# usc-isi/PipeEdge

Measured on NVIDIA H100. Metric: images/sec per pipeline, higher is better.
Workload: dtype f16

## Files before the change

### pipeedge_b200/csrc/gemm_wgmma.cu

```cuda
#include <math.h>
#include <stdio.h>
#include <stdlib.h>

#include "../../include/pipeedge_b200.h"
#include "common.cuh"
#include "ln_dev.cuh"
#include "wgmma.cuh"

namespace pe {

void count_launches(int n);
int require_sm90();

constexpr int kBlockM = 128;
constexpr int kBlockK = 64;
constexpr int kMmaK = 16;
constexpr int kNumConsumerWarps = 8;
constexpr int kConsumerThreads = kNumConsumerWarps * 32;
constexpr int kProducerWarp = kNumConsumerWarps;
constexpr int kWeightWarp = kNumConsumerWarps + 1;
constexpr int kGemmThreads = (kNumConsumerWarps + 2) * 32;
constexpr int kMaxStages = 8;
constexpr int kTraceSlots = 32;
constexpr int kPipeSmemBudget = 144 * 1024;
constexpr int kABytes = kBlockM * kBlockK * 2;

struct GemmParams {
  const float* bias;
  const float* resid;
  void* out;
  int m, n, k;
  int block_n;
  int stages;
  int num_m_blocks, num_n_blocks, num_k_blocks;
  long long* trace;
  int cm, cn;
  int num_super_m, num_super_n;
  int rows_per_item;
  int out_item_rows;
  int out_row_offset;
  int resid_per_item;
  int stg_offset;
  int static_w;
  int tma_out;
  const float* ln_gamma;
  const float* ln_beta;
  float ln_eps;
  int ln_off;
  int f32_is_ln;
  __half* out16;
};

constexpr int kLnAreaBytes = 8192;

__device__ __forceinline__ float gelu_erf(float x) { return 0.5f * x * (1.0f + erff(x * 0.70710678118654752f)); }
__device__ __forceinline__ float gelu_erf_fast(float x) {
  const float a = fminf(fabsf(x), 6.0f);
  float pl = fmaf(-1.889626233e-06f, a, 6.268140101e-05f);
  pl = fmaf(pl, a, -9.388679333e-04f);
  pl = fmaf(pl, a, 8.539461332e-03f);
  pl = fmaf(pl, a, -5.402068712e-02f);
  pl = fmaf(pl, a, -4.584097768e-01f);
  pl = fmaf(pl, a, -1.151269147e+00f);
  pl = fmaf(pl, a, -9.999943403e-01f);
  float e;
  asm("ex2.approx.ftz.f32 %0, %1;" : "=f"(e) : "f"(pl));
  return fmaxf(x, 0.0f) - fabsf(x * e);
}

constexpr int kStgLd = 36;
constexpr int kLnLdPad = 4;
constexpr int kStgBytesPerWarp = 16 * (128 + kLnLdPad) * 4;
constexpr int kStgBytes = kNumConsumerWarps * kStgBytesPerWarp;

__device__ __forceinline__ void map_rows(const GemmParams& p, int row, int& out_row, int& resid_row) {
  out_row = row;
  resid_row = row;
  if (p.rows_per_item > 0) {
    const int item = row / p.rows_per_item;
    const int in_item = row - item * p.rows_per_item + p.out_row_offset;
    out_row = item * p.out_item_rows + in_item;
    resid_row = p.resid_per_item ? in_item : out_row;
  }
}

template <int EPI>
__device__ __forceinline__ float epi_act(float x) {
  if (EPI == PE_EPI_GELU_F16) return gelu_erf_fast(x);
  if (EPI == PE_EPI_TANH_F32) return tanhf(x);
  return x;
}

template <int EPI>
__device__ __forceinline__ void epilogue_chunk16(const GemmParams& p, const float* stg, int row0, int col0, int lane) {
  constexpr bool kHalfOut = (EPI == PE_EPI_F16 || EPI == PE_EPI_GELU_F16);
  const bool vec_ok = (p.n & 7) == 0;
  if (kHalfOut) {
// ... 47 lines not shown
        if (row < p.m && fast) {
          int out_row, resid_row;
          map_rows(p, row, out_row, resid_row);
          res[it] = *reinterpret_cast<const float4*>(p.resid + static_cast<size_t>(resid_row) * p.n + col);
        }
      }
    }
    float4 bias4 = make_float4(0.f, 0.f, 0.f, 0.f);
    if (p.bias != nullptr && fast) bias4 = __ldg(reinterpret_cast<const float4*>(p.bias + col));
#pragma unroll
    for (int it = 0; it < 4; ++it) {
      const int rr = it * 4 + (lane >> 3);
      const int row = row0 + rr;
      if (row >= p.m || !col_ok) continue;
      int out_row, resid_row;
      map_rows(p, row, out_row, resid_row);
      const float4 a = *reinterpret_cast<const float4*>(stg + rr * kStgLd + cc);
      float* o = reinterpret_cast<float*>(p.out) + static_cast<size_t>(out_row) * p.n + col;
      if (fast) {
        float4 r4;
        r4.x = epi_act<EPI>(a.x + bias4.x) + res[it].x;
        r4.y = epi_act<EPI>(a.y + bias4.y) + res[it].y;
        r4.z = epi_act<EPI>(a.z + bias4.z) + res[it].z;
        r4.w = epi_act<EPI>(a.w + bias4.w) + res[it].w;
        *reinterpret_cast<float4*>(o) = r4;
      } else {
        const float v[4] = {a.x, a.y, a.z, a.w};
        for (int i = 0; i < 4 && col + i < p.n; ++i) {
          float x = v[i];
          if (p.bias != nullptr) x += __ldg(p.bias + col + i);
          x = epi_act<EPI>(x);
          if (EPI == PE_EPI_RESID_F32) x += p.resid[static_cast<size_t>(resid_row) * p.n + col + i];
          o[i] = x;
        }
      }
    }
  }
}

template <int J, int NACC>
__device__ __forceinline__ void stage_fragment(const float (&acc)[NACC], int j0, float* dst, int ld, int lane) {
  const int r = lane >> 2, c = (lane & 3) * 2;
#pragma unroll
  for (int j = 0; j < J; ++j) {
    *reinterpret_cast<float2*>(dst + r * ld + 8 * j + c) = make_float2(acc[4 * (j0 + j)], acc[4 * (j0 + j) + 1]);
    *reinterpret_cast<float2*>(dst + (r + 8) * ld + 8 * j + c) = make_float2(acc[4 * (j0 + j) + 2], acc[4 * (j0 + j) + 3]);
  }
}

constexpr int kWgStgBytes = 4 * kStgBytesPerWarp;
constexpr int kWgBoxBytes = 32 * 1024;
constexpr int kOutBoxCols = 32;

template <int EPI, int BN>
__device__ __forceinline__ void epilogue_tma(const GemmParams& p, const CUtensorMap* tm_c, const CUtensorMap* tm_r,
                                             const float (&acc)[BN / 2], uint8_t* stg, uint32_t stg_addr,
                                             uint32_t res_bar, uint32_t& res_phase, int row_wg, int col_tile, int wg,
                                             int lane, bool issuer) {
  constexpr bool kHalfOut = (EPI == PE_EPI_F16 || EPI == PE_EPI_GELU_F16);
  constexpr int kRowBytes = kOutBoxCols * (kHalfOut ? 2 : 4);
  constexpr int kBoxBytes = 64 * kRowBytes;
  constexpr int kBoxes = BN / kOutBoxCols;
  constexpr int kPass = kBoxes < kWgBoxBytes / kBoxBytes ? kBoxes : kWgBoxBytes / kBoxBytes;
  static_assert(kWgBoxBytes + 256 * 4 <= kWgStgBytes, "boxes + bias exceed a warpgroup's staging");
  float* bias_s = reinterpret_cast<float*>(stg + kWgBoxBytes);
  const int t = threadIdx.x & 127;
  const int r0 = (t >> 5) * 16 + (lane >> 2);
  const int cq = (lane & 3) * 2;
#pragma unroll
  for (int b0 = 0; b0 < kBoxes; b0 += kPass) {
    if (issuer) {
      tma_store_wait_read();
      if (EPI == PE_EPI_RESID_F32) {
        const int nb = (kBoxes - b0 < kPass ? kBoxes - b0 : kPass);
        int boxes = 0;
        if (row_wg < p.m)
          for (int b = 0; b < nb && col_tile + (b0 + b) * kOutBoxCols < p.n; ++b) boxes = b + 1;
        mbar_arrive_expect_tx_addr(res_bar, static_cast<uint32_t>(boxes * kBoxBytes));
        for (int b = 0; b < boxes; ++b)
          tma_load_2d_addr(stg_addr + static_cast<uint32_t>(b * kBoxBytes), tm_r, res_bar,
                           col_tile + (b0 + b) * kOutBoxCols, row_wg);
      }
    }
    if (b0 == 0) {
      for (int c = t; c < BN; c += 128) {
        const int col = col_tile + c;
        bias_s[c] = p.bias != nullptr && col < p.n ? __ldg(p.bias + col) : 0.f;
      }
    }
    named_barrier_id(3 + wg, 128);
    if (EPI == PE_EPI_RESID_F32) {
      mbar_wait_addr(res_bar, res_phase);
      res_phase ^= 1u;
    }
#pragma unroll
    for (int i = 0; i < kPass * 4; ++i) {
      const int j = b0 * 4 + i, jj = i & 3;
      if (j >= BN / 8) break;
      const float2 bv = *reinterpret_cast<const float2*>(bias_s + 8 * j + cq);
      uint8_t* box = stg + (i >> 2) * kBoxBytes;
#pragma unroll
      for (int h = 0; h < 2; ++h) {
        const int r = r0 + 8 * h;
        const float x0 = acc[4 * j + 2 * h] + bv.x, x1 = acc[4 * j + 2 * h + 1] + bv.y;
        if (kHalfOut) {
          *reinterpret_cast<__half2*>(box + r * kRowBytes + ((jj ^ ((r >> 1) & 3)) << 4) + cq * 2) =
              __floats2half2_rn(epi_act<EPI>(x0), epi_act<EPI>(x1));
        } else {
          float2* o = reinterpret_cast<float2*>(box + r * kRowBytes + (((2 * jj + (lane & 3) / 2) ^ (r & 7)) << 4) +
                                                (lane & 1) * 8);
          const float2 rv = EPI == PE_EPI_RESID_F32 ? *o : make_float2(0.f, 0.f);
          *o = make_float2(epi_act<EPI>(x0) + rv.x, epi_act<EPI>(x1) + rv.y);
        }
      }
    }
    fence_proxy_async_smem();
    named_barrier_id(3 + wg, 128);
    if (issuer) {
      if (row_wg < p.m) {
#pragma unroll
        for (int b = 0; b < kPass; ++b) {
          const int col = col_tile + (b0 + b) * kOutBoxCols;
          if (b0 + b < kBoxes && col < p.n) tma_store_2d(tm_c, stg_addr + static_cast<uint32_t>(b * kBoxBytes), col, row_wg);
        }
      }
      tma_store_commit();
    }
  }
}

template <int EPI, int BN>
__global__ void __launch_bounds__(kGemmThreads, 1)
gemm_wgmma_kernel(const __grid_constant__ CUtensorMap tm_a, const __grid_constant__ CUtensorMap tm_b,
                  const __grid_constant__ CUtensorMap tm_c, const __grid_constant__ CUtensorMap tm_r,
                  const GemmParams p) {
  extern __shared__ uint8_t smem_raw[];
  __shared__ __align__(8) uint64_t full_bar[kMaxStages];
  __shared__ __align__(8) uint64_t empty_bar[kMaxStages];
  __shared__ __align__(8) uint64_t ln_bar[2];
  __shared__ __align__(8) uint64_t res_bar[2];

  const int warp = threadIdx.x >> 5;
  const int lane = threadIdx.x & 31;
  long long* trace = p.trace != nullptr ? p.trace + static_cast<size_t>(blockIdx.x) * kTraceSlots : nullptr;
  if (trace != nullptr && threadIdx.x == 0) trace[0] = clock64();
  pdl_launch_dependents();
  const uint32_t smem_base = (smem_u32(smem_raw) + 1023u) & ~1023u;
  uint8_t* smem_gen = smem_raw + (smem_base - smem_u32(smem_raw));
  constexpr uint32_t stage_bytes = kABytes + static_cast<uint32_t>(BN) * (kBlockK * 2);

  const int csize = p.cm * p.cn;
  const uint32_t crank = csize > 1 ? cluster_ctarank() : 0u;
  const int m_rank = static_cast<int>(crank) % p.cm;
  const int n_rank = static_cast<int>(crank) / p.cm;
  uint16_t row_mask = 0, col_mask = 0;
  for (int c = 0; c < p.cn; ++c) row_mask |= static_cast<uint16_t>(1u << (m_rank + p.cm * c));
  for (int m = 0; m < p.cm; ++m) col_mask |= static_cast<uint16_t>(1u << (m + p.cm * n_rank));
  const uint16_t peers_mask = row_mask | col_mask;

  if (warp == kProducerWarp && lane == 0) {
    tma_prefetch_desc(&tm_a);
    tma_prefetch_desc(&tm_b);
    if (p.tma_out) tma_prefetch_desc(&tm_c);
    if (p.tma_out && EPI == PE_EPI_RESID_F32) tma_prefetch_desc(&tm_r);
    for (int s = 0; s < p.stages; ++s) {
      mbar_init(&full_bar[s], 1);
      mbar_init(&empty_bar[s], static_cast<uint32_t>(2 * (p.cm + p.cn - 1)));
    }
    for (int s = 0; s < 2; ++s) mbar_init(&ln_bar[s], static_cast<uint32_t>(p.cn));
    for (int s = 0; s < 2; ++s) mbar_init(&res_bar[s], 1);
    fence_barrier_init();
  }
  __syncthreads();
  if (csize > 1) cluster_sync_all();
  if (warp != kWeightWarp || p.static_w == 0) pdl_wait();
  if (trace != nullptr && threadIdx.x == 0) trace[1] = clock64();
  const int num_supers = p.num_super_m * p.num_super_n;
  const int cluster_id = static_cast<int>(blockIdx.x) / csize;
  const int num_clusters = static_cast<int>(gridDim.x) / csize;
  const int a_slice_rows = kBlockM / p.cn;
  const int b_slice_rows = p.block_n / p.cm;

  const uint32_t full_addr0 = keep_in_register(smem_u32(&full_bar[0]));
  const uint32_t empty_addr0 = keep_in_register(smem_u32(&empty_bar[0]));
  const int num_k_blocks = p.num_k_blocks, num_stages = p.stages;
  if (warp == kProducerWarp) {
    const int cm = p.cm, cn = p.cn, nsm = p.num_super_m;
    const uint32_t a_off = static_cast<uint32_t>(n_rank * a_slice_rows) * (kBlockK * 2);
    int stage = 0;
    uint32_t phase = 0;
    for (int sup = cluster_id; sup < num_supers; sup += num_clusters) {
      const int a_row = ((sup % nsm) * cm + m_rank) * kBlockM + n_rank * a_slice_rows;
      for (int kb = 0; kb < num_k_blocks; ++kb) {
        mbar_wait_addr(empty_addr0 + static_cast<uint32_t>(stage) * 8u, phase ^ 1u);
        if (elect_one()) {
          const uint32_t f = full_addr0 + static_cast<uint32_t>(stage) * 8u;
          const uint32_t sa = smem_base + static_cast<uint32_t>(stage) * stage_bytes + a_off;
          mbar_arrive_expect_tx_addr(f, stage_bytes);
          if (cn > 1) tma_load_2d_multicast_addr(sa, &tm_a, f, kb * kBlockK, a_row, row_mask);
          else tma_load_2d_addr(sa, &tm_a, f, kb * kBlockK, a_row);
        }
        __syncwarp();
        if (++stage == num_stages) { stage = 0; phase ^= 1u; }
      }
    }
  } else if (warp == kWeightWarp) {
    const int cm = p.cm, cn = p.cn, nsm = p.num_super_m, bn = p.block_n;
    const uint32_t b_off = kABytes + static_cast<uint32_t>(m_rank * b_slice_rows) * (kBlockK * 2);
    if (p.static_w != 0 && cluster_id < num_supers && elect_one()) {
      const int b_row = ((cluster_id / nsm) * cn + n_rank) * bn + m_rank * b_slice_rows;
      const int sharers = nsm * cm;
      const int me = (cluster_id % nsm) * cm + m_rank;
      for (int kb = num_stages + me; kb < num_k_blocks; kb += sharers) tma_prefetch_l2_2d(&tm_b, kb * kBlockK, b_row);
    }
    __syncwarp();
    int stage = 0;
    uint32_t phase = 0;
    for (int sup = cluster_id; sup < num_supers; sup += num_clusters) {
      const int b_row = ((sup / nsm) * cn + n_rank) * bn + m_rank * b_slice_rows;
      for (int kb = 0; kb < num_k_blocks; ++kb) {
        mbar_wait_addr(empty_addr0 + static_cast<uint32_t>(stage) * 8u, phase ^ 1u);
        if (elect_one()) {
          const uint32_t f = full_addr0 + static_cast<uint32_t>(stage) * 8u;
          const uint32_t sb = smem_base + static_cast<uint32_t>(stage) * stage_bytes + b_off;
          if (cm > 1) tma_load_2d_multicast_addr(sb, &tm_b, f, kb * kBlockK, b_row, col_mask);
          else tma_load_2d_addr(sb, &tm_b, f, kb * kBlockK, b_row);
        }
        __syncwarp();
        if (++stage == num_stages) { stage = 0; phase ^= 1u; }
      }
    }
  } else {
    const int wg = warp >> 2;
    const uint32_t a_wg_off = static_cast<uint32_t>(wg * 64) * (kBlockK * 2);
    const bool releaser = (warp & 3) == 0 && lane < csize && ((peers_mask >> lane) & 1u) != 0;
    const uint32_t empty_remote0 =
        csize > 1 ? mapa_shared(empty_addr0, static_cast<uint32_t>(lane < csize ? lane : 0)) : empty_addr0;
    float* stg = reinterpret_cast<float*>(smem_gen + p.stg_offset + warp * kStgBytesPerWarp);
    const bool store_issuer = (threadIdx.x & 127) == 0;
    const uint32_t res_bar_addr = smem_u32(&res_bar[wg]);
    uint32_t res_phase = 0u;
    int stage = 0;
    uint32_t phase = 0;
    int par = 0;
    uint32_t ln_phases = 0u;
    for (int sup = cluster_id; sup < num_supers; sup += num_clusters) {
      const int m_blk = (sup % p.num_super_m) * p.cm + m_rank;
      const int n_blk = (sup / p.num_super_m) * p.cn + n_rank;
      const int tslot = trace == nullptr || threadIdx.x != 0 ? -1 : (sup == cluster_id ? 0 : (sup == cluster_id + num_clusters ? 5 : -1));
      float acc[BN / 2];
#pragma unroll
      for (int i = 0; i < BN / 2; ++i) acc[i] = 0.f;
      int prev_stage = -1;
      for (int kb = 0; kb < num_k_blocks; ++kb) {
        mbar_wait_addr(full_addr0 + static_cast<uint32_t>(stage) * 8u, phase);
        if (tslot >= 0 && kb == 0) trace[2 + tslot] = clock64();
        const uint32_t sa = smem_base + static_cast<uint32_t>(stage) * stage_bytes;
        const uint64_t da = wgmma_desc_kmajor_sw128(sa + a_wg_off);
        const uint64_t db = wgmma_desc_kmajor_sw128(sa + kABytes);
        wgmma_fence();
#pragma unroll
        for (int k = 0; k < kBlockK / kMmaK; ++k)
          Wgmma<BN>::mma(acc, da + 2 * k, db + 2 * k, (kb | k) != 0 ? 1u : 0u);
        wgmma_commit();
        wgmma_wait<1>();
        if (prev_stage >= 0 && releaser) {
          const uint32_t e = empty_remote0 + static_cast<uint32_t>(prev_stage) * 8u;
          if (csize > 1) mbar_arrive_remote(e);
          else mbar_arrive_addr(e);
        }
        prev_stage = stage;
        if (++stage == num_stages) { stage = 0; phase ^= 1u; }
      }
      wgmma_wait<0>();
      if (releaser) {
        const uint32_t e = empty_remote0 + static_cast<uint32_t>(prev_stage) * 8u;
        if (csize > 1) mbar_arrive_remote(e);
        else mbar_arrive_addr(e);
      }
      if (tslot >= 0) trace[3 + tslot] = clock64();
      if (p.stg_offset == 0) named_barrier<1>(kConsumerThreads);
      const int row0 = m_blk * kBlockM + warp * 16;
      if (EPI == PE_EPI_RESID_LN) {
        constexpr int kLd = BN + kLnLdPad;
        constexpr int kChunks = BN / 32;
        float2* ln_part = reinterpret_cast<float2*>(smem_gen + p.ln_off);
        float2* ln_cta = ln_part + 4 * kBlockM;
        float2* ln_row = ln_cta + 2 * kBlockM;
        const int r_cta = warp * 16;
        const int gcol0 = n_blk * BN;
        stage_fragment<BN / 8>(acc, 0, stg, kLd, lane);
        __syncwarp();
        for (int idx = lane; idx < 16 * kChunks; idx += 32) {
          const int r = idx & 15, c = idx >> 4;
          const int row = row0 + r, gcol = gcol0 + c * 32;
          float* vr = stg + r * kLd + c * 32;
          float v[32];
          if (row < p.m) {
            const float4* r4 = reinterpret_cast<const float4*>(p.resid + static_cast<size_t>(row) * p.n + gcol);
            const float4* b4 = reinterpret_cast<const float4*>(p.bias + gcol);
#pragma unroll
            for (int i = 0; i < 8; ++i) {
// ... 12 lines not shown
          for (int i = 0; i < 8; ++i)
            *reinterpret_cast<float4*>(vr + 4 * i) = make_float4(v[4 * i], v[4 * i + 1], v[4 * i + 2], v[4 * i + 3]);
          float mean_c, m2_c;
          ln_chunk32(v, mean_c, m2_c);
          ln_part[(r_cta + r) * 4 + c] = make_float2(mean_c, m2_c);
        }
        __syncwarp();
        if (lane < 16) {
          const float2 q0 = ln_part[(r_cta + lane) * 4];
          float cnt = 32.f, mean = q0.x, m2 = q0.y;
          for (int c = 1; c < kChunks; ++c) {
            const float2 q = ln_part[(r_cta + lane) * 4 + c];
            ln_merge(cnt, mean, m2, 32.f, q.x, q.y);
          }
          ln_cta[par * kBlockM + r_cta + lane] = make_float2(mean, m2);
        }
        named_barrier<2>(kConsumerThreads);
        if (warp == 0 && lane < p.cn)
          mbar_arrive_cluster(mapa_shared(smem_u32(&ln_bar[par]), static_cast<uint32_t>(lane)));
        mbar_wait_cluster(&ln_bar[par], (ln_phases >> par) & 1u);
        ln_phases ^= 1u << par;
        if (lane < 16) {
          float cnt = 0.f, mean = 0.f, m2 = 0.f;
          const uint32_t mine = smem_u32(&ln_cta[par * kBlockM + r_cta + lane]);
          const float bn = static_cast<float>(p.block_n);
          for (int j = 0; j < p.cn; ++j) {
            const float2 q = ld_dsmem_f2(mapa_shared(mine, static_cast<uint32_t>(j)));
            ln_merge(cnt, mean, m2, bn, q.x, q.y);
          }
          ln_row[r_cta + lane] = make_float2(mean, ln_rstd(m2, 1.0f / static_cast<float>(p.n), p.ln_eps));
        }
        __syncwarp();
        if (lane < BN / 4) {
          const int gcol = gcol0 + lane * 4;
          const float4 g4 = __ldg(reinterpret_cast<const float4*>(p.ln_gamma + gcol));
          const float4 e4 = __ldg(reinterpret_cast<const float4*>(p.ln_beta + gcol));
          for (int r = 0; r < 16 && row0 + r < p.m; ++r) {
            const float4 v = *reinterpret_cast<const float4*>(stg + r * kLd + lane * 4);
            const float2 st = ln_row[r_cta + r];
            const float4 ln = make_float4(ln_apply(v.x, st.x, st.y, g4.x, e4.x), ln_apply(v.y, st.x, st.y, g4.y, e4.y),
                                          ln_apply(v.z, st.x, st.y, g4.z, e4.z), ln_apply(v.w, st.x, st.y, g4.w, e4.w));
            const size_t off = static_cast<size_t>(row0 + r) * p.n + gcol;
            if (p.out != nullptr) *reinterpret_cast<float4*>(static_cast<float*>(p.out) + off) = p.f32_is_ln ? ln : v;
            if (p.out16 != nullptr) {
              uint2 pk;
              __half2* h2 = reinterpret_cast<__half2*>(&pk);
              h2[0] = __floats2half2_rn(ln.x, ln.y);
              h2[1] = __floats2half2_rn(ln.z, ln.w);
              *reinterpret_cast<uint2*>(p.out16 + off) = pk;
            }
          }
        }
        par ^= 1;
      } else if (p.tma_out) {
        const uint32_t wg_stg = static_cast<uint32_t>(p.stg_offset + wg * kWgStgBytes);
        epilogue_tma<EPI, BN>(p, &tm_c, &tm_r, acc, smem_gen + wg_stg, smem_base + wg_stg, res_bar_addr, res_phase,
                              m_blk * kBlockM + wg * 64, n_blk * BN, wg, lane, store_issuer);
      } else {
#pragma unroll
        for (int c = 0; c < BN / 32; ++c) {
          const int col0 = n_blk * BN + c * 32;
          stage_fragment<4>(acc, 4 * c, stg, kStgLd, lane);
          __syncwarp();
          if (row0 < p.m && col0 < p.n) epilogue_chunk16<EPI>(p, stg, row0, col0, lane);
          __syncwarp();
        }
      }
      if (tslot >= 0) trace[5 + tslot] = clock64();
    }
    if (p.tma_out && store_issuer) tma_store_wait_all();
  }

  __syncthreads();
  if (csize > 1) cluster_sync_all();
  if (trace != nullptr && threadIdx.x == 0) trace[6] = clock64();
}

typedef CUresult (*EncodeTiledFn)(CUtensorMap*, CUtensorMapDataType, cuuint32_t, void*, const cuuint64_t*,
                                  const cuuint64_t*, const cuuint32_t*, const cuuint32_t*, CUtensorMapInterleave,
                                  CUtensorMapSwizzle, CUtensorMapL2promotion, CUtensorMapFloatOOBfill);

static EncodeTiledFn get_encode_fn() {
  static EncodeTiledFn fn = nullptr;
  if (fn == nullptr) {
    void* ptr = nullptr;
    cudaDriverEntryPointQueryResult qres;
    if (cudaGetDriverEntryPoint("cuTensorMapEncodeTiled", &ptr, cudaEnableDefault, &qres) != cudaSuccess ||
        qres != cudaDriverEntryPointSuccess || ptr == nullptr) {
      set_error("cuTensorMapEncodeTiled is not available from the driver");
      return nullptr;
    }
    fn = reinterpret_cast<EncodeTiledFn>(ptr);
  }
  return fn;
}

static int encode_f16_2d(CUtensorMap* map, const void* ptr, uint64_t rows, uint64_t cols, uint32_t box_rows) {
  EncodeTiledFn fn = get_encode_fn();
  if (fn == nullptr) return PE_ERR_CUDA;
  const cuuint64_t dims[2] = {cols, rows};
  const cuuint64_t strides[1] = {cols * 2};
  const cuuint32_t box[2] = {kBlockK, box_rows};
  const cuuint32_t estr[2] = {1, 1};
  const CUresult rc = fn(map, CU_TENSOR_MAP_DATA_TYPE_FLOAT16, 2, const_cast<void*>(ptr), dims, strides, box, estr,
                         CU_TENSOR_MAP_INTERLEAVE_NONE, CU_TENSOR_MAP_SWIZZLE_128B, CU_TENSOR_MAP_L2_PROMOTION_L2_256B,
                         CU_TENSOR_MAP_FLOAT_OOB_FILL_NONE);
  if (rc != CUDA_SUCCESS) {
    set_error("cuTensorMapEncodeTiled failed (CUresult %d) for [%llu x %llu] box %u", static_cast<int>(rc),
              static_cast<unsigned long long>(rows), static_cast<unsigned long long>(cols), box_rows);
    return PE_ERR_CUDA;
  }
  return PE_OK;
}

static int encode_out_2d(CUtensorMap* map, void* ptr, uint64_t rows, uint64_t cols, bool half) {
  EncodeTiledFn fn = get_encode_fn();
  if (fn == nullptr) return PE_ERR_CUDA;
  const uint64_t esize = half ? 2 : 4;
  const cuuint64_t dims[2] = {cols, rows};
  const cuuint64_t strides[1] = {cols * esize};
  const cuuint32_t box[2] = {kOutBoxCols, 64};
  const cuuint32_t estr[2] = {1, 1};
  const CUresult rc = fn(map, half ? CU_TENSOR_MAP_DATA_TYPE_FLOAT16 : CU_TENSOR_MAP_DATA_TYPE_FLOAT32, 2, ptr, dims,
                         strides, box, estr, CU_TENSOR_MAP_INTERLEAVE_NONE,
                         half ? CU_TENSOR_MAP_SWIZZLE_64B : CU_TENSOR_MAP_SWIZZLE_128B, CU_TENSOR_MAP_L2_PROMOTION_NONE,
                         CU_TENSOR_MAP_FLOAT_OOB_FILL_NONE);
  if (rc != CUDA_SUCCESS) {
    set_error("cuTensorMapEncodeTiled failed (CUresult %d) for the [%llu x %llu] GEMM output", static_cast<int>(rc),
              static_cast<unsigned long long>(rows), static_cast<unsigned long long>(cols));
    return PE_ERR_CUDA;
  }
  return PE_OK;
}

static bool gemm_tma_store_enabled() {
  static const bool on = [] {
    const char* e = getenv("PE_GEMM_REG_STORE");
    return !(e != nullptr && e[0] == '1');
  }();
  return on;
}

static long long* g_gemm_trace = nullptr;
void set_gemm_trace(void* buf) { g_gemm_trace = static_cast<long long*>(buf); }

struct GemmPlan {
  int cm, cn, bn;
};

static int max_clusters(int csize) {
  return csize == 1 ? kNumSMs : (csize == 2 ? kNumSMs / 2 : 128 / csize);
}

GemmPlan plan_gemm(int m, int n, int k, int epilogue) {
  int forced[3] = {0, 0, 0};
  const char* env = getenv("PE_GEMM_FORCE");
  if (env != nullptr && sscanf(env, "%d,%d,%d", &forced[0], &forced[1], &forced[2]) == 3 && forced[0] > 0)
    return {forced[0], forced[1], forced[2]};
  GemmPlan best = {1, 1, 32};
  double best_cost = 1e30;
  const double kb = (k + kBlockK - 1) / kBlockK;
  const double epi_per_col = epilogue == PE_EPI_GELU_F16 ? 14.0 : (epilogue == PE_EPI_TANH_F32 ? 16.0
                             : (epilogue == PE_EPI_RESID_F32 ? 6.0 : 4.0));
  for (int bn = 256; bn >= 32; bn -= 32) {
    const long tiles = static_cast<long>((m + kBlockM - 1) / kBlockM) * ((n + bn - 1) / bn);
    const long rounds = (tiles + kNumSMs - 1) / kNumSMs;
    const double cost = 3000.0 + rounds * (kb * (150.0 + 4.0 * bn) + 800.0 + epi_per_col * bn);
    if (cost < best_cost - 1e-9) {
      best_cost = cost;
      best = {1, 1, bn};
    }
  }
  const int m_blocks = (m + kBlockM - 1) / kBlockM, n_blocks = (n + best.bn - 1) / best.bn;
  const bool pairs_one_wave = static_cast<long>(m_blocks) * ((n_blocks + 1) / 2) <= max_clusters(2);
  if (kb >= 32 && pairs_one_wave && (64.0 + best.bn) < 0.75 * (128.0 + best.bn)) best = {1, 2, best.bn};
  return best;
}

template <int EPI, int BN>
static int launch_gemm(const CUtensorMap& ta, const CUtensorMap& tb, const CUtensorMap& tc, const CUtensorMap& tr,
                       const GemmParams& p, cudaStream_t stream) {
  static bool configured = false;
  const int max_smem = kPipeSmemBudget + kStgBytes + kLnAreaBytes + 1024;
  if (!configured) {
    PE_CUDA(cudaFuncSetAttribute(gemm_wgmma_kernel<EPI, BN>, cudaFuncAttributeMaxDynamicSharedMemorySize, max_smem));
    configured = true;
  }
  const uint32_t stage_bytes = kABytes + static_cast<uint32_t>(p.block_n) * (kBlockK * 2);
  const size_t ring = static_cast<size_t>(p.stages) * stage_bytes, stg_end = static_cast<size_t>(p.stg_offset) + kStgBytes;
  size_t smem = (ring > stg_end ? ring : stg_end) + 1024;
  if (EPI == PE_EPI_RESID_LN) smem = static_cast<size_t>(p.ln_off) + kLnAreaBytes + 1024;
  const int csize = p.cm * p.cn;
  const int supers = p.num_super_m * p.num_super_n;
  const int avail = max_clusters(csize);
  const int clusters = supers < avail ? supers : avail;
  cudaLaunchConfig_t cfg = {};
  cfg.gridDim = dim3(static_cast<unsigned>(clusters * csize));
  cfg.blockDim = dim3(kGemmThreads);
  cfg.dynamicSmemBytes = smem;
  cfg.stream = stream;
  cudaLaunchAttribute attr[2];
  attr[0].id = cudaLaunchAttributeClusterDimension;
  attr[0].val.clusterDim.x = static_cast<unsigned>(csize);
  attr[0].val.clusterDim.y = 1;
  attr[0].val.clusterDim.z = 1;
  attr[1].id = cudaLaunchAttributeProgrammaticStreamSerialization;
  attr[1].val.programmaticStreamSerializationAllowed = 1;
  cfg.attrs = attr;
  cfg.numAttrs = pdl_enabled() ? 2 : 1;
  PE_CUDA(cudaLaunchKernelEx(&cfg, gemm_wgmma_kernel<EPI, BN>, ta, tb, tc, tr, p));
  count_launches(1);
  return PE_OK;
}

template <int EPI, int kMaxBN = 256>
static int launch_gemm_bn(const CUtensorMap& ta, const CUtensorMap& tb, const CUtensorMap& tc, const CUtensorMap& tr,
                          const GemmParams& p, cudaStream_t stream) {
  switch (p.block_n) {
    case 32: return launch_gemm<EPI, 32>(ta, tb, tc, tr, p, stream);
    case 64: return launch_gemm<EPI, 64>(ta, tb, tc, tr, p, stream);
    case 96: return launch_gemm<EPI, 96>(ta, tb, tc, tr, p, stream);
    case 128: return launch_gemm<EPI, 128>(ta, tb, tc, tr, p, stream);
    default: break;
  }
  if constexpr (kMaxBN > 128) {
    switch (p.block_n) {
      case 160: return launch_gemm<EPI, 160>(ta, tb, tc, tr, p, stream);
      case 192: return launch_gemm<EPI, 192>(ta, tb, tc, tr, p, stream);
      case 224: return launch_gemm<EPI, 224>(ta, tb, tc, tr, p, stream);
      case 256: return launch_gemm<EPI, 256>(ta, tb, tc, tr, p, stream);
      default: break;
    }
  }
  set_error("pe_linear: no kernel for block_n=%d", p.block_n);
  return PE_ERR_INVALID;
}

static void fill_geometry(GemmParams& p, const GemmPlan& plan, int m, int n, int k, int reserve = 0) {
  p.m = m; p.n = n; p.k = k;
  p.block_n = plan.bn;
  p.cm = plan.cm;
  p.cn = plan.cn;
  const uint32_t stage_bytes = kABytes + static_cast<uint32_t>(p.block_n) * (kBlockK * 2);
  p.num_m_blocks = (m + kBlockM - 1) / kBlockM;
  p.num_n_blocks = (n + p.block_n - 1) / p.block_n;
  p.num_super_m = (p.num_m_blocks + p.cm - 1) / p.cm;
  p.num_super_n = (p.num_n_blocks + p.cn - 1) / p.cn;
  const bool one_round = p.num_super_m * p.num_super_n <= max_clusters(p.cm * p.cn);
  int stages = ((one_round ? kPipeSmemBudget + kStgBytes : kPipeSmemBudget) - reserve) / static_cast<int>(stage_bytes);
  p.stages = stages > kMaxStages ? kMaxStages : (stages < 2 ? 2 : stages);
  if (const char* cap = getenv("PE_GEMM_STAGES")) {
    const int c = atoi(cap);
    if (c >= 2 && c < p.stages) p.stages = c;
  }
  p.stg_offset = one_round ? 0 : p.stages * static_cast<int>(stage_bytes);
  p.num_k_blocks = (k + kBlockK - 1) / kBlockK;
}

int linear_impl(const void* a, const void* w, const void* bias, const void* resid, void* out, int m, int n, int k,
                int epilogue, int rows_per_item, int out_item_rows, int out_row_offset, int resid_per_item,
                int static_w, cudaStream_t stream) {
  PE_REQUIRE(a && w && out, "pe_linear: null pointer");
  PE_REQUIRE(m > 0 && n > 0 && k > 0, "pe_linear: bad shape m=%d n=%d k=%d", m, n, k);
  PE_REQUIRE((k & 7) == 0, "pe_linear: k=%d must be a multiple of 8 (16-byte TMA row pitch)", k);
  PE_REQUIRE((reinterpret_cast<uintptr_t>(a) & 15) == 0 && (reinterpret_cast<uintptr_t>(w) & 15) == 0,
             "pe_linear: operands must be 16-byte aligned");
  PE_REQUIRE(epilogue != PE_EPI_RESID_F32 || resid != nullptr, "pe_linear: PE_EPI_RESID_F32 needs resid");
  int rc = require_sm90();
  if (rc != PE_OK) return rc;

  const GemmPlan plan = plan_gemm(m, n, k, epilogue);
  PE_REQUIRE(plan.bn >= 32 && plan.bn <= 256 && plan.bn % 32 == 0 && plan.cm >= 1 && plan.cn >= 1 &&
                 plan.cm * plan.cn <= 8 && kBlockM % plan.cn == 0 && (plan.bn / plan.cm) % 8 == 0,
             "pe_linear: bad tile plan cm=%d cn=%d bn=%d", plan.cm, plan.cn, plan.bn);
  GemmParams p = {};
  p.bias = static_cast<const float*>(bias);
  p.resid = static_cast<const float*>(resid);
  p.out = out;
  fill_geometry(p, plan, m, n, k);
  p.trace = g_gemm_trace;
  p.rows_per_item = rows_per_item;
  p.out_item_rows = out_item_rows;
  p.out_row_offset = out_row_offset;
  p.resid_per_item = resid_per_item;
  p.static_w = static_w != 0 ? 1 : 0;

  CUtensorMap ta, tb;
  rc = encode_f16_2d(&ta, a, static_cast<uint64_t>(m), static_cast<uint64_t>(k), static_cast<uint32_t>(kBlockM / p.cn));
  if (rc != PE_OK) return rc;
  rc = encode_f16_2d(&tb, w, static_cast<uint64_t>(n), static_cast<uint64_t>(k), static_cast<uint32_t>(p.block_n / p.cm));
  if (rc != PE_OK) return rc;
  CUtensorMap tc = {}, tr = {};
  const bool half_out = epilogue == PE_EPI_F16 || epilogue == PE_EPI_GELU_F16;
  p.tma_out = gemm_tma_store_enabled() && rows_per_item == 0 && (n & 7) == 0 &&
              (reinterpret_cast<uintptr_t>(out) & 15) == 0 && (resid == nullptr || (reinterpret_cast<uintptr_t>(resid) & 15) == 0);
  if (p.tma_out) {
    rc = encode_out_2d(&tc, out, static_cast<uint64_t>(m), static_cast<uint64_t>(n), half_out);
    if (rc != PE_OK) return rc;
    if (epilogue == PE_EPI_RESID_F32) {
      rc = encode_out_2d(&tr, const_cast<void*>(resid), static_cast<uint64_t>(m), static_cast<uint64_t>(n), false);
      if (rc != PE_OK) return rc;
    }
  }
  switch (epilogue) {
    case PE_EPI_F16: return launch_gemm_bn<PE_EPI_F16>(ta, tb, tc, tr, p, stream);
    case PE_EPI_GELU_F16: return launch_gemm_bn<PE_EPI_GELU_F16>(ta, tb, tc, tr, p, stream);
    case PE_EPI_RESID_F32: return launch_gemm_bn<PE_EPI_RESID_F32>(ta, tb, tc, tr, p, stream);
    case PE_EPI_F32: return launch_gemm_bn<PE_EPI_F32>(ta, tb, tc, tr, p, stream);
    case PE_EPI_TANH_F32: return launch_gemm_bn<PE_EPI_TANH_F32>(ta, tb, tc, tr, p, stream);
    default: set_error("pe_linear: unknown epilogue %d", epilogue); return PE_ERR_INVALID;
  }
}

int linear_ln_cluster(int n) {
  for (int cn = 8; cn >= 1; cn >>= 1)
    if (n % cn == 0 && (n / cn) % 32 == 0 && n / cn <= 128 && kBlockM % cn == 0) return cn;
  return 0;
}

int linear_ln_impl(const void* a, const void* w, const void* bias, const void* resid, const void* gamma, const void* beta,
                   float eps, void* out_f32, int f32_is_ln, void* out_f16, int m, int n, int k, int static_w,
                   cudaStream_t stream) {
  PE_REQUIRE(a && w && bias && resid && gamma && beta && (out_f32 || out_f16), "pe_linear_residual_layernorm: null pointer");
  PE_REQUIRE(m > 0 && n > 0 && k > 0 && (k & 7) == 0, "pe_linear_residual_layernorm: bad shape m=%d n=%d k=%d", m, n, k);
  const int cn = linear_ln_cluster(n);
  PE_REQUIRE(cn > 0, "pe_linear_residual_layernorm: n=%d is not supported (needs n = cn * bn, cn in {1,2,4,8}, bn %% 32 == 0, bn <= 128)", n);
  PE_REQUIRE((reinterpret_cast<uintptr_t>(a) & 15) == 0 && (reinterpret_cast<uintptr_t>(w) & 15) == 0 &&
                 (reinterpret_cast<uintptr_t>(resid) & 15) == 0 && (reinterpret_cast<uintptr_t>(bias) & 15) == 0 &&
                 (reinterpret_cast<uintptr_t>(gamma) & 15) == 0 && (reinterpret_cast<uintptr_t>(beta) & 15) == 0 &&
                 (out_f32 == nullptr || (reinterpret_cast<uintptr_t>(out_f32) & 15) == 0) &&
                 (out_f16 == nullptr || (reinterpret_cast<uintptr_t>(out_f16) & 15) == 0),
             "pe_linear_residual_layernorm: operands must be 16-byte aligned");
  int rc = require_sm90();
  if (rc != PE_OK) return rc;
  const GemmPlan plan = {1, cn, n / cn};
  GemmParams p = {};
  p.bias = static_cast<const float*>(bias);
  p.resid = static_cast<const float*>(resid);
  p.out = out_f32;
  p.out16 = static_cast<__half*>(out_f16);
  fill_geometry(p, plan, m, n, k, kLnAreaBytes);
  p.trace = nullptr;
  p.static_w = static_w != 0 ? 1 : 0;
  p.ln_gamma = static_cast<const float*>(gamma);
  p.ln_beta = static_cast<const float*>(beta);
  p.ln_eps = eps;
  p.f32_is_ln = f32_is_ln;
  {
    const uint32_t stage_bytes = kABytes + static_cast<uint32_t>(p.block_n) * (kBlockK * 2);
    const size_t ring = static_cast<size_t>(p.stages) * stage_bytes, stg_end = static_cast<size_t>(p.stg_offset) + kStgBytes;
    p.ln_off = static_cast<int>(((ring > stg_end ? ring : stg_end) + 1023) / 1024 * 1024);
  }
  CUtensorMap ta, tb;
  rc = encode_f16_2d(&ta, a, static_cast<uint64_t>(m), static_cast<uint64_t>(k), static_cast<uint32_t>(kBlockM / p.cn));
  if (rc != PE_OK) return rc;
  rc = encode_f16_2d(&tb, w, static_cast<uint64_t>(n), static_cast<uint64_t>(k), static_cast<uint32_t>(p.block_n));
  if (rc != PE_OK) return rc;
  const CUtensorMap tc = {}, tr = {};
  return launch_gemm_bn<PE_EPI_RESID_LN, 128>(ta, tb, tc, tr, p, stream);
}

int gemm_plan_query(int m, int n, int k, int epilogue, int* out6) {
  PE_REQUIRE(out6 != nullptr && m > 0 && n > 0 && k > 0, "pe_debug_gemm_plan: bad arguments");
  PE_REQUIRE(epilogue >= PE_EPI_F16 && epilogue <= PE_EPI_TANH_F32, "pe_debug_gemm_plan: unknown epilogue %d", epilogue);
  const GemmPlan plan = plan_gemm(m, n, k, epilogue);
  GemmParams p = {};
  fill_geometry(p, plan, m, n, k);
  const int supers = p.num_super_m * p.num_super_n, avail = max_clusters(p.cm * p.cn);
  out6[0] = p.cm; out6[1] = p.cn; out6[2] = p.block_n; out6[3] = p.stages;
  out6[4] = p.num_m_blocks * p.num_n_blocks;
  out6[5] = (supers < avail ? supers : avail) * p.cm * p.cn;
  return PE_OK;
}

template <int EPI>
__global__ void gemm_simt_kernel(const __half* __restrict__ a, const __half* __restrict__ w,
                                 const float* __restrict__ bias, const float* resid, void* out, int m, int n, int k) {
  __shared__ float sa[16][17];
  __shared__ float sw[16][17];
  const int tx = threadIdx.x, ty = threadIdx.y;
  const int row = blockIdx.y * 16 + ty, col = blockIdx.x * 16 + tx;
  float acc = 0.f;
  for (int k0 = 0; k0 < k; k0 += 16) {
    const int ar = blockIdx.y * 16 + ty, ac = k0 + tx;
    sa[ty][tx] = (ar < m && ac < k) ? __half2float(a[static_cast<size_t>(ar) * k + ac]) : 0.f;
    const int wr = blockIdx.x * 16 + ty, wc = k0 + tx;
    sw[ty][tx] = (wr < n && wc < k) ? __half2float(w[static_cast<size_t>(wr) * k + wc]) : 0.f;
    __syncthreads();
// ... 39 lines not shown
```

Before: 7741.

## Add dedicated epilogue warpgroup with smem accumulator hand-off for multi-wave GEMMs

Adds a fourth, epilogue-only warpgroup to the GEMM kernel. Consumer warpgroups write their accumulators to a double-buffered shared-memory hand-off area and return to the next tile's MMA main loop, while the epilogue warpgroup applies bias/activation/residual and issues the TMA stores. It is enabled only for single-CTA plans whose tile count falls between one and two waves, so the epilogue of one tile overlaps the mainloop of the next. Bias loads are hoisted into registers before the mainloop, and the residual reads are batched ahead of the writes. In exchange it uses more threads and shared memory, which can reduce pipeline stages, and it adds an extra smem round trip for the accumulators.

Result: faster. 7909, median of 6 (+2.2%).

```diff
diff --git a/pipeedge_b200/csrc/gemm_wgmma.cu b/pipeedge_b200/csrc/gemm_wgmma.cu
--- a/pipeedge_b200/csrc/gemm_wgmma.cu
+++ b/pipeedge_b200/csrc/gemm_wgmma.cu
@@ -20,6 +20,13 @@
 constexpr int kProducerWarp = kNumConsumerWarps;
 constexpr int kWeightWarp = kNumConsumerWarps + 1;
 constexpr int kGemmThreads = (kNumConsumerWarps + 2) * 32;
+constexpr int kEpiWarp0 = kNumConsumerWarps + 2;
+constexpr int kHandoffThreads = kGemmThreads + 128;
+constexpr int kHandoffMaxBN = 160;
+constexpr int handoff_max_bn(int epi) { return epi == PE_EPI_RESID_F32 ? 128 : kHandoffMaxBN; }
+constexpr int kEpiBarrier = 5;
+constexpr int kSmemPerBlock = 227 * 1024;
+constexpr int kStaticSmemMax = 256;
 constexpr int kMaxStages = 8;
 constexpr int kTraceSlots = 32;
 constexpr int kPipeSmemBudget = 144 * 1024;
@@ -43,6 +50,7 @@
   int stg_offset;
   int static_w;
   int tma_out;
+  int handoff;
   const float* ln_gamma;
   const float* ln_beta;
   float ln_eps;
@@ -196,18 +204,25 @@
 constexpr int kWgBoxBytes = 32 * 1024;
 constexpr int kOutBoxCols = 32;
 
-template <int EPI, int BN>
+template <int BN>
+__device__ __forceinline__ float2 tile_bias(const GemmParams& p, int col_tile, int t) {
+  float2 b = make_float2(0.f, 0.f);
+  if (p.bias != nullptr && t < BN && col_tile + t < p.n) b.x = __ldg(p.bias + col_tile + t);
+  if (p.bias != nullptr && t + 128 < BN && col_tile + t + 128 < p.n) b.y = __ldg(p.bias + col_tile + t + 128);
+  return b;
+}
+
+template <int EPI, int BN, int kBoxArea>
 __device__ __forceinline__ void epilogue_tma(const GemmParams& p, const CUtensorMap* tm_c, const CUtensorMap* tm_r,
                                              const float (&acc)[BN / 2], uint8_t* stg, uint32_t stg_addr,
-                                             uint32_t res_bar, uint32_t& res_phase, int row_wg, int col_tile, int wg,
-                                             int lane, bool issuer) {
+                                             float* bias_s, float2 bias_r, uint32_t res_bar, uint32_t& res_phase, int row_wg,
+                                             int col_tile, int bar_id, int lane, bool issuer) {
   constexpr bool kHalfOut = (EPI == PE_EPI_F16 || EPI == PE_EPI_GELU_F16);
   constexpr int kRowBytes = kOutBoxCols * (kHalfOut ? 2 : 4);
   constexpr int kBoxBytes = 64 * kRowBytes;
   constexpr int kBoxes = BN / kOutBoxCols;
-  constexpr int kPass = kBoxes < kWgBoxBytes / kBoxBytes ? kBoxes : kWgBoxBytes / kBoxBytes;
-  static_assert(kWgBoxBytes + 256 * 4 <= kWgStgBytes, "boxes + bias exceed a warpgroup's staging");
-  float* bias_s = reinterpret_cast<float*>(stg + kWgBoxBytes);
+  constexpr int kPass = kBoxes < kBoxArea / kBoxBytes ? kBoxes : kBoxArea / kBoxBytes;
+  static_assert(kPass >= 1, "the staging holds no output box");
   const int t = threadIdx.x & 127;
   const int r0 = (t >> 5) * 16 + (lane >> 2);
   const int cq = (lane & 3) * 2;
@@ -227,39 +242,52 @@
       }
     }
     if (b0 == 0) {
-      for (int c = t; c < BN; c += 128) {
-        const int col = col_tile + c;
-        bias_s[c] = p.bias != nullptr && col < p.n ? __ldg(p.bias + col) : 0.f;
-      }
-    }
-    named_barrier_id(3 + wg, 128);
+      if (t < BN) bias_s[t] = bias_r.x;
+      if (t + 128 < BN) bias_s[t + 128] = bias_r.y;
+    }
+    named_barrier_id(bar_id, 128);
     if (EPI == PE_EPI_RESID_F32) {
       mbar_wait_addr(res_bar, res_phase);
       res_phase ^= 1u;
     }
 #pragma unroll
-    for (int i = 0; i < kPass * 4; ++i) {
-      const int j = b0 * 4 + i, jj = i & 3;
-      if (j >= BN / 8) break;
-      const float2 bv = *reinterpret_cast<const float2*>(bias_s + 8 * j + cq);
-      uint8_t* box = stg + (i >> 2) * kBoxBytes;
-#pragma unroll
-      for (int h = 0; h < 2; ++h) {
-        const int r = r0 + 8 * h;
-        const float x0 = acc[4 * j + 2 * h] + bv.x, x1 = acc[4 * j + 2 * h + 1] + bv.y;
-        if (kHalfOut) {
-          *reinterpret_cast<__half2*>(box + r * kRowBytes + ((jj ^ ((r >> 1) & 3)) << 4) + cq * 2) =
-              __floats2half2_rn(epi_act<EPI>(x0), epi_act<EPI>(x1));
-        } else {
-          float2* o = reinterpret_cast<float2*>(box + r * kRowBytes + (((2 * jj + (lane & 3) / 2) ^ (r & 7)) << 4) +
-                                                (lane & 1) * 8);
-          const float2 rv = EPI == PE_EPI_RESID_F32 ? *o : make_float2(0.f, 0.f);
-          *o = make_float2(epi_act<EPI>(x0) + rv.x, epi_act<EPI>(x1) + rv.y);
+    for (int bx = 0; bx < kPass; ++bx) {
+      const int j0 = (b0 + bx) * 4;
+      if (j0 >= BN / 8) break;
+      uint8_t* box = stg + bx * kBoxBytes;
+      float2 bv[4], rv[4][2];
+#pragma unroll
+      for (int jj = 0; jj < 4; ++jj) {
+        bv[jj] = *reinterpret_cast<const float2*>(bias_s + 8 * (j0 + jj) + cq);
+#pragma unroll
+        for (int h = 0; h < 2; ++h) {
+          const int r = r0 + 8 * h;
+          rv[jj][h] = EPI == PE_EPI_RESID_F32
+                          ? *reinterpret_cast<const float2*>(box + r * kRowBytes +
+                                                             (((2 * jj + (lane & 3) / 2) ^ (r & 7)) << 4) + (lane & 1) * 8)
+                          : make_float2(0.f, 0.f);
+        }
+      }
+#pragma unroll
+      for (int jj = 0; jj < 4; ++jj) {
+        const int j = j0 + jj;
+#pragma unroll
+        for (int h = 0; h < 2; ++h) {
+          const int r = r0 + 8 * h;
+          const float x0 = acc[4 * j + 2 * h] + bv[jj].x, x1 = acc[4 * j + 2 * h + 1] + bv[jj].y;
+          if (kHalfOut) {
+            *reinterpret_cast<__half2*>(box + r * kRowBytes + ((jj ^ ((r >> 1) & 3)) << 4) + cq * 2) =
+                __floats2half2_rn(epi_act<EPI>(x0), epi_act<EPI>(x1));
+          } else {
+            *reinterpret_cast<float2*>(box + r * kRowBytes + (((2 * jj + (lane & 3) / 2) ^ (r & 7)) << 4) +
+                                       (lane & 1) * 8) =
+                make_float2(epi_act<EPI>(x0) + rv[jj][h].x, epi_act<EPI>(x1) + rv[jj][h].y);
+          }
         }
       }
     }
     fence_proxy_async_smem();
-    named_barrier_id(3 + wg, 128);
+    named_barrier_id(bar_id, 128);
     if (issuer) {
       if (row_wg < p.m) {
 #pragma unroll
@@ -273,8 +301,24 @@
   }
 }
 
-template <int EPI, int BN>
-__global__ void __launch_bounds__(kGemmThreads, 1)
+template <int BN>
+__device__ __forceinline__ void handoff_write(float* buf, const float (&acc)[BN / 2], int t) {
+#pragma unroll
+  for (int q = 0; q < BN / 8; ++q)
+    *reinterpret_cast<float4*>(buf + q * 512 + 4 * t) = make_float4(acc[4 * q], acc[4 * q + 1], acc[4 * q + 2], acc[4 * q + 3]);
+}
+
+template <int BN>
+__device__ __forceinline__ void handoff_read(const float* buf, float (&acc)[BN / 2], int t) {
+#pragma unroll
+  for (int q = 0; q < BN / 8; ++q) {
+    const float4 v = *reinterpret_cast<const float4*>(buf + q * 512 + 4 * t);
+    acc[4 * q] = v.x; acc[4 * q + 1] = v.y; acc[4 * q + 2] = v.z; acc[4 * q + 3] = v.w;
+  }
+}
+
+template <int EPI, int BN, bool HANDOFF>
+__global__ void __launch_bounds__(HANDOFF ? kHandoffThreads : kGemmThreads, 1)
 gemm_wgmma_kernel(const __grid_constant__ CUtensorMap tm_a, const __grid_constant__ CUtensorMap tm_b,
                   const __grid_constant__ CUtensorMap tm_c, const __grid_constant__ CUtensorMap tm_r,
                   const GemmParams p) {
@@ -282,7 +326,9 @@
   __shared__ __align__(8) uint64_t full_bar[kMaxStages];
   __shared__ __align__(8) uint64_t empty_bar[kMaxStages];
   __shared__ __align__(8) uint64_t ln_bar[2];
-  __shared__ __align__(8) uint64_t res_bar[2];
+  __shared__ __align__(8) uint64_t res_bar[3];
+  __shared__ __align__(8) uint64_t hand_full[2];
+  __shared__ __align__(8) uint64_t hand_empty[2];
 
   const int warp = threadIdx.x >> 5;
   const int lane = threadIdx.x & 31;
@@ -292,6 +338,7 @@
   const uint32_t smem_base = (smem_u32(smem_raw) + 1023u) & ~1023u;
   uint8_t* smem_gen = smem_raw + (smem_base - smem_u32(smem_raw));
   constexpr uint32_t stage_bytes = kABytes + static_cast<uint32_t>(BN) * (kBlockK * 2);
+  constexpr int kHandoffBoxArea = 256 * BN < kWgBoxBytes ? 256 * BN : kWgBoxBytes;
 
   const int csize = p.cm * p.cn;
   const uint32_t crank = csize > 1 ? cluster_ctarank() : 0u;
@@ -312,7 +359,13 @@
       mbar_init(&empty_bar[s], static_cast<uint32_t>(2 * (p.cm + p.cn - 1)));
     }
     for (int s = 0; s < 2; ++s) mbar_init(&ln_bar[s], static_cast<uint32_t>(p.cn));
-    for (int s = 0; s < 2; ++s) mbar_init(&res_bar[s], 1);
+    for (int s = 0; s < 3; ++s) mbar_init(&res_bar[s], 1);
+    if (HANDOFF) {
+      for (int s = 0; s < 2; ++s) {
+        mbar_init(&hand_full[s], 128);
+        mbar_init(&hand_empty[s], 1);
+      }
+    }
     fence_barrier_init();
   }
   __syncthreads();
@@ -374,6 +427,37 @@
         if (++stage == num_stages) { stage = 0; phase ^= 1u; }
       }
     }
+  } else if (HANDOFF && warp >= kEpiWarp0) {
+    const bool issuer = threadIdx.x == kEpiWarp0 * 32;
+    const int t = threadIdx.x & 127;
+    uint32_t hphase = 0u, res_phase = 0u;
+    int tile_i = 0;
+    for (int sup = cluster_id; sup + num_clusters < num_supers; sup += num_clusters, ++tile_i) {
+      const int m_blk = sup % p.num_super_m, n_blk = sup / p.num_super_m;
+      const int eslot = trace == nullptr || !issuer ? -1 : (tile_i < 2 ? 11 + 2 * tile_i : -1);
+      const float2 bias_r = tile_bias<BN>(p, n_blk * BN, t);
+#pragma unroll 1
+      for (int g = 0; g < 2; ++g) {
+        const uint32_t buf_off = static_cast<uint32_t>(p.stg_offset + g * 256 * BN);
+        float* buf = reinterpret_cast<float*>(smem_gen + buf_off);
+        mbar_wait_addr(smem_u32(&hand_full[g]), hphase);
+        if (eslot >= 0 && g == 0) trace[eslot] = clock64();
+        float acc[BN / 2];
+        handoff_read<BN>(buf, acc, t);
+        named_barrier_id(kEpiBarrier, 128);
+        epilogue_tma<EPI, BN, kHandoffBoxArea>(p, &tm_c, &tm_r, acc, smem_gen + buf_off, smem_base + buf_off,
+                                        reinterpret_cast<float*>(smem_gen + p.stg_offset + 512 * BN + g * 4 * BN),
+                                        bias_r, smem_u32(&res_bar[2]), res_phase, m_blk * kBlockM + g * 64, n_blk * BN,
+                                        kEpiBarrier, lane, issuer);
+        if (issuer) {
+          tma_store_wait_read();
+          mbar_arrive_addr(smem_u32(&hand_empty[g]));
+        }
+      }
+      hphase ^= 1u;
+      if (eslot >= 0) trace[eslot + 1] = clock64();
+    }
+    if (issuer) tma_store_wait_all();
   } else {
     const int wg = warp >> 2;
     const uint32_t a_wg_off = static_cast<uint32_t>(wg * 64) * (kBlockK * 2);
@@ -384,6 +468,7 @@
     const bool store_issuer = (threadIdx.x & 127) == 0;
     const uint32_t res_bar_addr = smem_u32(&res_bar[wg]);
     uint32_t res_phase = 0u;
+    uint32_t hphase = 0u;
     int stage = 0;
     uint32_t phase = 0;
     int par = 0;
@@ -392,6 +477,8 @@
       const int m_blk = (sup % p.num_super_m) * p.cm + m_rank;
       const int n_blk = (sup / p.num_super_m) * p.cn + n_rank;
       const int tslot = trace == nullptr || threadIdx.x != 0 ? -1 : (sup == cluster_id ? 0 : (sup == cluster_id + num_clusters ? 5 : -1));
+      const float2 bias_r = p.tma_out && EPI != PE_EPI_RESID_LN ? tile_bias<BN>(p, n_blk * BN, threadIdx.x & 127)
+                                                                 : make_float2(0.f, 0.f);
       float acc[BN / 2];
 #pragma unroll
       for (int i = 0; i < BN / 2; ++i) acc[i] = 0.f;
@@ -510,10 +597,24 @@
           }
         }
         par ^= 1;
+      } else if (HANDOFF) {
+        const uint32_t buf_off = static_cast<uint32_t>(p.stg_offset + wg * 256 * BN);
+        mbar_wait_addr(smem_u32(&hand_empty[wg]), hphase ^ 1u);
+        hphase ^= 1u;
+        if (sup + num_clusters < num_supers) {
+          handoff_write<BN>(reinterpret_cast<float*>(smem_gen + buf_off), acc, threadIdx.x & 127);
+          mbar_arrive_addr(smem_u32(&hand_full[wg]));
+        } else {
+          epilogue_tma<EPI, BN, kHandoffBoxArea>(p, &tm_c, &tm_r, acc, smem_gen + buf_off, smem_base + buf_off,
+                                          reinterpret_cast<float*>(smem_gen + p.stg_offset + 512 * BN + wg * 4 * BN),
+                                          bias_r, res_bar_addr, res_phase, m_blk * kBlockM + wg * 64, n_blk * BN, 3 + wg, lane,
+                                          store_issuer);
+        }
       } else if (p.tma_out) {
         const uint32_t wg_stg = static_cast<uint32_t>(p.stg_offset + wg * kWgStgBytes);
-        epilogue_tma<EPI, BN>(p, &tm_c, &tm_r, acc, smem_gen + wg_stg, smem_base + wg_stg, res_bar_addr, res_phase,
-                              m_blk * kBlockM + wg * 64, n_blk * BN, wg, lane, store_issuer);
+        epilogue_tma<EPI, BN, kWgBoxBytes>(p, &tm_c, &tm_r, acc, smem_gen + wg_stg, smem_base + wg_stg,
+                                           reinterpret_cast<float*>(smem_gen + wg_stg + kWgBoxBytes), bias_r, res_bar_addr,
+                                           res_phase, m_blk * kBlockM + wg * 64, n_blk * BN, 3 + wg, lane, store_issuer);
       } else {
 #pragma unroll
         for (int c = 0; c < BN / 32; ++c) {
@@ -604,18 +705,30 @@
 
 struct GemmPlan {
   int cm, cn, bn;
+  int handoff;
 };
 
 static int max_clusters(int csize) {
   return csize == 1 ? kNumSMs : (csize == 2 ? kNumSMs / 2 : 128 / csize);
 }
 
+static int handoff_extra_smem(int bn) { return 512 * bn + 8 * bn + 1024 + kStaticSmemMax; }
+
+static bool handoff_fits(int m, int n, int epilogue, const GemmPlan& plan) {
+  const long tiles = static_cast<long>((m + kBlockM - 1) / kBlockM) * ((n + plan.bn - 1) / plan.bn);
+  return plan.cm == 1 && plan.cn == 1 && plan.bn <= handoff_max_bn(epilogue) && tiles > kNumSMs &&
+         tiles <= 2 * kNumSMs;
+}
+
 GemmPlan plan_gemm(int m, int n, int k, int epilogue) {
-  int forced[3] = {0, 0, 0};
+  int forced[4] = {0, 0, 0, -1};
   const char* env = getenv("PE_GEMM_FORCE");
-  if (env != nullptr && sscanf(env, "%d,%d,%d", &forced[0], &forced[1], &forced[2]) == 3 && forced[0] > 0)
-    return {forced[0], forced[1], forced[2]};
-  GemmPlan best = {1, 1, 32};
+  if (env != nullptr && sscanf(env, "%d,%d,%d,%d", &forced[0], &forced[1], &forced[2], &forced[3]) >= 3 && forced[0] > 0) {
+    GemmPlan f = {forced[0], forced[1], forced[2], 0};
+    f.handoff = forced[3] >= 0 ? (forced[3] != 0 ? 1 : 0) : (handoff_fits(m, n, epilogue, f) ? 1 : 0);
+    return f;
+  }
+  GemmPlan best = {1, 1, 32, 0};
   double best_cost = 1e30;
   const double kb = (k + kBlockK - 1) / kBlockK;
   const double epi_per_col = epilogue == PE_EPI_GELU_F16 ? 14.0 : (epilogue == PE_EPI_TANH_F32 ? 16.0
@@ -626,35 +739,43 @@
     const double cost = 3000.0 + rounds * (kb * (150.0 + 4.0 * bn) + 800.0 + epi_per_col * bn);
     if (cost < best_cost - 1e-9) {
       best_cost = cost;
-      best = {1, 1, bn};
+      best = {1, 1, bn, 0};
     }
   }
   const int m_blocks = (m + kBlockM - 1) / kBlockM, n_blocks = (n + best.bn - 1) / best.bn;
   const bool pairs_one_wave = static_cast<long>(m_blocks) * ((n_blocks + 1) / 2) <= max_clusters(2);
-  if (kb >= 32 && pairs_one_wave && (64.0 + best.bn) < 0.75 * (128.0 + best.bn)) best = {1, 2, best.bn};
+  if (kb >= 32 && pairs_one_wave && (64.0 + best.bn) < 0.75 * (128.0 + best.bn)) best = {1, 2, best.bn, 0};
+  best.handoff = handoff_fits(m, n, epilogue, best) ? 1 : 0;
   return best;
 }
 
-template <int EPI, int BN>
+template <int EPI, int BN, bool HANDOFF>
 static int launch_gemm(const CUtensorMap& ta, const CUtensorMap& tb, const CUtensorMap& tc, const CUtensorMap& tr,
                        const GemmParams& p, cudaStream_t stream) {
   static bool configured = false;
-  const int max_smem = kPipeSmemBudget + kStgBytes + kLnAreaBytes + 1024;
+  const int max_smem = HANDOFF ? kSmemPerBlock - kStaticSmemMax : kPipeSmemBudget + kStgBytes + kLnAreaBytes + 1024;
   if (!configured) {
-    PE_CUDA(cudaFuncSetAttribute(gemm_wgmma_kernel<EPI, BN>, cudaFuncAttributeMaxDynamicSharedMemorySize, max_smem));
+    cudaFuncAttributes fa;
+    PE_CUDA(cudaFuncGetAttributes(&fa, gemm_wgmma_kernel<EPI, BN, HANDOFF>));
+    PE_REQUIRE(fa.sharedSizeBytes <= static_cast<size_t>(kStaticSmemMax), "pe_linear: %zu bytes of static shared memory",
+               fa.sharedSizeBytes);
+    PE_CUDA(cudaFuncSetAttribute(gemm_wgmma_kernel<EPI, BN, HANDOFF>, cudaFuncAttributeMaxDynamicSharedMemorySize, max_smem));
     configured = true;
   }
   const uint32_t stage_bytes = kABytes + static_cast<uint32_t>(p.block_n) * (kBlockK * 2);
   const size_t ring = static_cast<size_t>(p.stages) * stage_bytes, stg_end = static_cast<size_t>(p.stg_offset) + kStgBytes;
   size_t smem = (ring > stg_end ? ring : stg_end) + 1024;
   if (EPI == PE_EPI_RESID_LN) smem = static_cast<size_t>(p.ln_off) + kLnAreaBytes + 1024;
+  if (HANDOFF) smem = ring + static_cast<size_t>(handoff_extra_smem(BN) - kStaticSmemMax);
+  PE_REQUIRE(smem <= static_cast<size_t>(max_smem), "pe_linear: the plan needs %zu bytes of shared memory (BN %d, %d stages)",
+             smem + kStaticSmemMax, BN, p.stages);
   const int csize = p.cm * p.cn;
   const int supers = p.num_super_m * p.num_super_n;
   const int avail = max_clusters(csize);
   const int clusters = supers < avail ? supers : avail;
   cudaLaunchConfig_t cfg = {};
   cfg.gridDim = dim3(static_cast<unsigned>(clusters * csize));
-  cfg.blockDim = dim3(kGemmThreads);
+  cfg.blockDim = dim3(HANDOFF ? kHandoffThreads : kGemmThreads);
   cfg.dynamicSmemBytes = smem;
   cfg.stream = stream;
   cudaLaunchAttribute attr[2];
@@ -666,7 +787,7 @@
   attr[1].val.programmaticStreamSerializationAllowed = 1;
   cfg.attrs = attr;
   cfg.numAttrs = pdl_enabled() ? 2 : 1;
-  PE_CUDA(cudaLaunchKernelEx(&cfg, gemm_wgmma_kernel<EPI, BN>, ta, tb, tc, tr, p));
+  PE_CUDA(cudaLaunchKernelEx(&cfg, gemm_wgmma_kernel<EPI, BN, HANDOFF>, ta, tb, tc, tr, p));
   count_launches(1);
   return PE_OK;
 }
@@ -674,19 +795,35 @@
 template <int EPI, int kMaxBN = 256>
 static int launch_gemm_bn(const CUtensorMap& ta, const CUtensorMap& tb, const CUtensorMap& tc, const CUtensorMap& tr,
                           const GemmParams& p, cudaStream_t stream) {
+  if constexpr (EPI != PE_EPI_RESID_LN) {
+    if (p.handoff) {
+      switch (p.block_n) {
+        case 32: return launch_gemm<EPI, 32, true>(ta, tb, tc, tr, p, stream);
+        case 64: return launch_gemm<EPI, 64, true>(ta, tb, tc, tr, p, stream);
+        case 96: return launch_gemm<EPI, 96, true>(ta, tb, tc, tr, p, stream);
+        case 128: return launch_gemm<EPI, 128, true>(ta, tb, tc, tr, p, stream);
+        case 160:
+          if constexpr (handoff_max_bn(EPI) >= 160) return launch_gemm<EPI, 160, true>(ta, tb, tc, tr, p, stream);
+          [[fallthrough]];
+        default: set_error("pe_linear: no epilogue hand-off kernel for block_n=%d (at most %d)", p.block_n,
+                           handoff_max_bn(EPI));
+                 return PE_ERR_INVALID;
+      }
+    }
+  }
   switch (p.block_n) {
-    case 32: return launch_gemm<EPI, 32>(ta, tb, tc, tr, p, stream);
-    case 64: return launch_gemm<EPI, 64>(ta, tb, tc, tr, p, stream);
-    case 96: return launch_gemm<EPI, 96>(ta, tb, tc, tr, p, stream);
-    case 128: return launch_gemm<EPI, 128>(ta, tb, tc, tr, p, stream);
+    case 32: return launch_gemm<EPI, 32, false>(ta, tb, tc, tr, p, stream);
+    case 64: return launch_gemm<EPI, 64, false>(ta, tb, tc, tr, p, stream);
+    case 96: return launch_gemm<EPI, 96, false>(ta, tb, tc, tr, p, stream);
+    case 128: return launch_gemm<EPI, 128, false>(ta, tb, tc, tr, p, stream);
     default: break;
   }
   if constexpr (kMaxBN > 128) {
     switch (p.block_n) {
-      case 160: return launch_gemm<EPI, 160>(ta, tb, tc, tr, p, stream);
-      case 192: return launch_gemm<EPI, 192>(ta, tb, tc, tr, p, stream);
-      case 224: return launch_gemm<EPI, 224>(ta, tb, tc, tr, p, stream);
-      case 256: return launch_gemm<EPI, 256>(ta, tb, tc, tr, p, stream);
+      case 160: return launch_gemm<EPI, 160, false>(ta, tb, tc, tr, p, stream);
+      case 192: return launch_gemm<EPI, 192, false>(ta, tb, tc, tr, p, stream);
+      case 224: return launch_gemm<EPI, 224, false>(ta, tb, tc, tr, p, stream);
+      case 256: return launch_gemm<EPI, 256, false>(ta, tb, tc, tr, p, stream);
       default: break;
     }
   }
@@ -705,14 +842,20 @@
   p.num_super_m = (p.num_m_blocks + p.cm - 1) / p.cm;
   p.num_super_n = (p.num_n_blocks + p.cn - 1) / p.cn;
   const bool one_round = p.num_super_m * p.num_super_n <= max_clusters(p.cm * p.cn);
-  int stages = ((one_round ? kPipeSmemBudget + kStgBytes : kPipeSmemBudget) - reserve) / static_cast<int>(stage_bytes);
+  int budget = (one_round ? kPipeSmemBudget + kStgBytes : kPipeSmemBudget) - reserve;
+  if (plan.handoff) {
+    const int room = kSmemPerBlock - handoff_extra_smem(plan.bn);
+    budget = room < budget ? room : budget;
+  }
+  int stages = budget / static_cast<int>(stage_bytes);
   p.stages = stages > kMaxStages ? kMaxStages : (stages < 2 ? 2 : stages);
   if (const char* cap = getenv("PE_GEMM_STAGES")) {
     const int c = atoi(cap);
     if (c >= 2 && c < p.stages) p.stages = c;
   }
-  p.stg_offset = one_round ? 0 : p.stages * static_cast<int>(stage_bytes);
+  p.stg_offset = one_round && !plan.handoff ? 0 : p.stages * static_cast<int>(stage_bytes);
   p.num_k_blocks = (k + kBlockK - 1) / kBlockK;
+  p.handoff = plan.handoff;
 }
 
 int linear_impl(const void* a, const void* w, const void* bias, const void* resid, void* out, int m, int n, int k,
@@ -731,6 +874,9 @@
   PE_REQUIRE(plan.bn >= 32 && plan.bn <= 256 && plan.bn % 32 == 0 && plan.cm >= 1 && plan.cn >= 1 &&
                  plan.cm * plan.cn <= 8 && kBlockM % plan.cn == 0 && (plan.bn / plan.cm) % 8 == 0,
              "pe_linear: bad tile plan cm=%d cn=%d bn=%d", plan.cm, plan.cn, plan.bn);
+  PE_REQUIRE(!plan.handoff || (plan.cm == 1 && plan.cn == 1 && plan.bn <= handoff_max_bn(epilogue)),
+             "pe_linear: the epilogue hand-off needs single CTAs and BN <= %d for this epilogue: cm=%d cn=%d bn=%d",
+             handoff_max_bn(epilogue), plan.cm, plan.cn, plan.bn);
   GemmParams p = {};
   p.bias = static_cast<const float*>(bias);
   p.resid = static_cast<const float*>(resid);
@@ -760,6 +906,7 @@
       if (rc != PE_OK) return rc;
     }
   }
+  p.handoff = p.handoff && p.tma_out ? 1 : 0;
   switch (epilogue) {
     case PE_EPI_F16: return launch_gemm_bn<PE_EPI_F16>(ta, tb, tc, tr, p, stream);
     case PE_EPI_GELU_F16: return launch_gemm_bn<PE_EPI_GELU_F16>(ta, tb, tc, tr, p, stream);
@@ -791,7 +938,7 @@
              "pe_linear_residual_layernorm: operands must be 16-byte aligned");
   int rc = require_sm90();
   if (rc != PE_OK) return rc;
-  const GemmPlan plan = {1, cn, n / cn};
+  const GemmPlan plan = {1, cn, n / cn, 0};
   GemmParams p = {};
   p.bias = static_cast<const float*>(bias);
   p.resid = static_cast<const float*>(resid);
```
